# liuxinren456852/HiDeGS

Measured on NVIDIA B200. Metric: fwd+bwd Mpix/s @1M Gaussians 1080p, higher is better.
Workload: dtype f32

## Files before the change

### hidegs_b200/csrc/blend_bwd.cu

```cuda
#include "blend_common.cuh"

#include <cstdlib>
#include <mutex>

namespace hg {

namespace {

constexpr int kThreadsB = 128;


struct PixelState {
  float w[9];
  float bgT, T, acc_g, last_g, last_alpha;
  int last_contributor;
};

struct PairState {
  float2 w[9];
  float2 bgT, T, acc_g, last_g, last_alpha;
  int lastA, lastB;
};

template <int HALF>
__device__ __forceinline__ float& half_of(float2& v) { return HALF ? v.y : v.x; }
template <int HALF>
__device__ __forceinline__ float half_of(const float2& v) { return HALF ? v.y : v.x; }

template <bool GEO, bool DEPTH>
__device__ __forceinline__ void load_pixel_state(PixelState& s, bool inside, size_t pix, size_t HW, int W, int H,
                                                 float pixx, float pixy, float fx, float fy, int n,
                                                 const float* __restrict__ bg_color,
                                                 const float* __restrict__ all_map_pixels,
                                                 const float* __restrict__ final_Ts,
                                                 const uint32_t* __restrict__ n_contrib,
                                                 const float* __restrict__ dL_dpixels,
                                                 const float* __restrict__ dL_dout_all_maps,
                                                 const float* __restrict__ dL_dout_plane_depths,
                                                 const float* __restrict__ dL_invdepths) {
#pragma unroll
  for (int i = 0; i < 9; ++i) s.w[i] = 0.f;
  const float T_final = inside ? final_Ts[pix] : 0.f;
  s.last_contributor = inside ? min((int)n_contrib[pix], n) : 0;
  float bg_dot = 0.f;
  if (inside) {
#pragma unroll
    for (int c = 0; c < 3; ++c) {
      s.w[c] = dL_dpixels[c * HW + pix];
      bg_dot += __ldg(bg_color + c) * s.w[c];
    }
    if (DEPTH) s.w[3] = dL_invdepths[pix];
    if (GEO) {
#pragma unroll
      for (int c = 0; c < 5; ++c) s.w[4 + c] = dL_dout_all_maps[c * HW + pix];
      const float rayx = (float)(((double)pixx - W * 0.5) / (double)fx);
      const float rayy = (float)(((double)pixy - H * 0.5) / (double)fy);
      const float nx = all_map_pixels[pix], ny = all_map_pixels[HW + pix], nz = all_map_pixels[2 * HW + pix];
      const float dist = all_map_pixels[4 * HW + pix];
      const float tmp = (float)((double)(nx * rayx + ny * rayy + nz) + 1.0e-8);
      const float dpd = dL_dout_plane_depths[pix];
      s.w[8] += (-dpd / tmp);
      s.w[4] += dpd * (dist / (tmp * tmp) * rayx);
      s.w[5] += dpd * (dist / (tmp * tmp) * rayy);
      s.w[6] += dpd * (dist / (tmp * tmp));
    }
  }
  s.bgT = -T_final * bg_dot;
  s.T = T_final;
  s.acc_g = s.last_g = s.last_alpha = 0.f;
}

constexpr int kGroupC = 16;
constexpr int kWarpsC = kThreadsB / 32;

constexpr int kRecQuadsC = 4;
constexpr int kAStride = 68;

template <bool INTERP>
struct alignas(16) BwdMmaSmem {
  float4 rec[kWarpsC][32 * kRecQuadsC];
  alignas(16) float a_w[kWarpsC][kGroupC * kAStride];
  float a_p[kWarpsC][kGroupC * kAStride];
  float2 b_ch0[kWarpsC][8][32];
  float2 b_ch8[kWarpsC][8][4];
  float2 zero2;
  float2 b_mom[8][32];
  float2 tf[INTERP ? kWarpsC : 1][INTERP ? 32 : 1];
  uint32_t info[kWarpsC][32];
};
constexpr uint32_t kHasA = 1u << 30, kHasB = 1u << 31;
constexpr uint32_t kARowBytes = kAStride * 4;
constexpr uint32_t kAPOffset = kWarpsC * kGroupC * kAStride * 4;
constexpr uint32_t kMetaOffset = 64 * 4;

__device__ __forceinline__ void sts_v2(uint32_t addr, float a, float b) {
  asm volatile("st.shared.v2.f32 [%0], {%1, %2};" ::"r"(addr), "f"(a), "f"(b) : "memory");
}
__device__ __forceinline__ void sts_v4(uint32_t addr, float a, float b, float c, float d) {
  asm volatile("st.shared.v4.f32 [%0], {%1, %2, %3, %4};" ::"r"(addr), "f"(a), "f"(b), "f"(c), "f"(d) : "memory");
}

__device__ __forceinline__ void ldmatrix_x4(uint32_t (&r)[4], const float* smem_row_ptr) {
  const uint32_t a = (uint32_t)__cvta_generic_to_shared(smem_row_ptr);
  asm volatile("ldmatrix.sync.aligned.m8n8.x4.shared.b16 {%0,%1,%2,%3}, [%4];"
               : "=r"(r[0]), "=r"(r[1]), "=r"(r[2]), "=r"(r[3])
               : "r"(a));
}

__device__ __forceinline__ void split_tf32(float v, uint32_t& hi, uint32_t& lo) {
  asm("and.b32 %0, %1, 0xffffe000;" : "=r"(hi) : "r"(__float_as_uint(v)));
  lo = __float_as_uint(v - __uint_as_float(hi));
}

__device__ __forceinline__ void split_tf32_pair(float v0, float v1, uint32_t& hi0, uint32_t& lo0, uint32_t& hi1,
                                                uint32_t& lo1) {
  asm("and.b32 %0, %1, 0xffffe000;" : "=r"(hi0) : "r"(__float_as_uint(v0)));
  asm("and.b32 %0, %1, 0xffffe000;" : "=r"(hi1) : "r"(__float_as_uint(v1)));
  const float2 lo = __fadd2_rn(make_float2(v0, v1), make_float2(-__uint_as_float(hi0), -__uint_as_float(hi1)));
  lo0 = __float_as_uint(lo.x);
  lo1 = __float_as_uint(lo.y);
}

__device__ __forceinline__ void mma_tf32(float (&d)[4], uint32_t a0, uint32_t a1, uint32_t a2, uint32_t a3, uint32_t b0,
                                         uint32_t b1) {
  asm volatile(
      "mma.sync.aligned.m16n8k8.row.col.f32.tf32.tf32.f32 {%0,%1,%2,%3}, {%4,%5,%6,%7}, {%8,%9}, {%0,%1,%2,%3};"
      : "+f"(d[0]), "+f"(d[1]), "+f"(d[2]), "+f"(d[3])
      : "r"(a0), "r"(a1), "r"(a2), "r"(a3), "r"(b0), "r"(b1));
}

__device__ __forceinline__ void red_add_v2(float* p, float a, float b) {
  asm volatile("red.global.add.v2.f32 [%0], {%1, %2};" ::"l"(p), "f"(a), "f"(b) : "memory");
}
__device__ __forceinline__ void red_add_v4(float* p, float a, float b, float c, float d) {
  asm volatile("red.global.add.v4.f32 [%0], {%1, %2, %3, %4};" ::"l"(p), "f"(a), "f"(b), "f"(c), "f"(d) : "memory");
}

template <bool GEO, bool DEPTH, bool INTERP, bool ACC, int HALF>
__device__ __forceinline__ bool pixel_pair_c(PairState& ps, const float4 ea, const float4 eb, const float4 ec,
                                             const float4 ed, const float2 tf, float pixx, float2 neg_pixy, int q,
                                             float& wgt, float& p, float& p3, bool& near) {
  struct {
    float &T, &acc_g, &last_g, &last_alpha;
    const float bgT;
    const int last_contributor;
    float w[9];
  } s{half_of<HALF>(ps.T), half_of<HALF>(ps.acc_g), half_of<HALF>(ps.last_g), half_of<HALF>(ps.last_alpha),
      half_of<HALF>(ps.bgT), HALF ? ps.lastB : ps.lastA,
      {half_of<HALF>(ps.w[0]), half_of<HALF>(ps.w[1]), half_of<HALF>(ps.w[2]), half_of<HALF>(ps.w[3]),
       half_of<HALF>(ps.w[4]), half_of<HALF>(ps.w[5]), half_of<HALF>(ps.w[6]), half_of<HALF>(ps.w[7]),
       half_of<HALF>(ps.w[8])}};
  const float dx = __fsub_rn(ea.x, pixx), dy = __fadd_rn(ea.y, half_of<HALF>(neg_pixy));
  const float quad = __fmaf_rn(dx, __fmul_rn(dx, ea.z), __fmul_rn(dy, __fmul_rn(dy, eb.x)));
  const float power = __fmaf_rn(quad, -0.5f, -__fmul_rn(dy, __fmul_rn(dx, ea.w)));
  const float test_alpha = __fmul_rn(eb.y, expf(power));
  float blend_alpha = fminf(0.99f, test_alpha);
  float opac_mult = 1.0f;
  if (INTERP) {
    const float my_alpha = blend_alpha;
    if (ACC) {
      const float kidsqrt = 1.0f - powf(1.0f - my_alpha, tf.y);
      blend_alpha = tf.x * my_alpha + (1.0f - tf.x) * kidsqrt;
      opac_mult = tf.x - powf(1.0f - my_alpha, tf.y - 1.0f) * (tf.x - 1.0f) * tf.y;
    } else {
      const float lg = __log2f(1.0f - my_alpha);
      const float kidsqrt = 1.0f - exp2f(tf.y * lg);
      blend_alpha = tf.x * my_alpha + (1.0f - tf.x) * kidsqrt;
      opac_mult = tf.x - exp2f((tf.y - 1.0f) * lg) * (tf.x - 1.0f) * tf.y;
      near = near || fabsf(blend_alpha - 1.0f / 255.0f) < 2e-6f;
    }
  }
  const bool valid = (q < s.last_contributor) && !(power > 0.0f) && !(blend_alpha < 1.0f / 255.0f);
  const float alpha = valid ? blend_alpha : 0.f;
  float rinv;
  asm("rcp.approx.ftz.f32 %0, %1;" : "=f"(rinv) : "f"(1.0f - alpha));
  const float Tn = s.T * rinv;
  wgt = alpha * Tn;
  float g = ec.x * s.w[0] + ec.y * s.w[1] + ec.z * s.w[2];
  if (DEPTH) g += ec.w * s.w[3];
  if (GEO) {
    const float ee = eb.z;
    g += ed.x * s.w[4] + ed.y * s.w[5] + ed.z * s.w[6] + ed.w * s.w[7] + ee * s.w[8];
  }
  const float acc_new = s.last_alpha * s.last_g + (1.0f - s.last_alpha) * s.acc_g;
  const float dL_dalpha = (g - acc_new) * Tn + s.bgT * rinv;
  s.T = Tn;
  s.acc_g = acc_new;
  s.last_g = g;
  s.last_alpha = alpha;
  p = test_alpha > 0.99f ? 0.f : (INTERP ? (valid ? test_alpha : 0.f) : alpha) * dL_dalpha;
  p3 = INTERP ? opac_mult * p : 0.f;
  return valid;
}

template <bool GEO, bool DEPTH>
__device__ __forceinline__ bool pixel_pair_c2(PairState& s, const float4 ea, const float4 eb, const float4 ec,
                                              const float4 ed, float pixx, float2 neg_pixy, int q, float2& wgt,
                                              float2& p) {
  const float dx = __fsub_rn(ea.x, pixx);
  const float dxa = __fmul_rn(dx, ea.z);
  const float ndxb = __fmul_rn(dx, -ea.w);
  const float2 dy = __fadd2_rn(bc2(ea.y), neg_pixy);
  const float2 quad = __ffma2_rn(bc2(dx), bc2(dxa), __fmul2_rn(dy, __fmul2_rn(dy, bc2(eb.x))));
  const float2 power = __ffma2_rn(quad, bc2(-0.5f), __fmul2_rn(dy, bc2(ndxb)));
  const float2 test_alpha = __fmul2_rn(bc2(eb.y), expf_pair(power));
  const float bA = fminf(0.99f, test_alpha.x), bB = fminf(0.99f, test_alpha.y);
  const bool validA = (q < s.lastA) && !(power.x > 0.0f) && !(bA < 1.0f / 255.0f);
  const bool validB = (q < s.lastB) && !(power.y > 0.0f) && !(bB < 1.0f / 255.0f);
  const float2 alpha = make_float2(validA ? bA : 0.f, validB ? bB : 0.f);
  const float2 om = __ffma2_rn(alpha, bc2(-1.0f), bc2(1.0f));
  float2 rinv;
  asm("rcp.approx.ftz.f32 %0, %1;" : "=f"(rinv.x) : "f"(om.x));
  asm("rcp.approx.ftz.f32 %0, %1;" : "=f"(rinv.y) : "f"(om.y));
  const float2 Tn = __fmul2_rn(s.T, rinv);
  wgt = __fmul2_rn(alpha, Tn);
  float2 g = __ffma2_rn(bc2(ec.z), s.w[2], __ffma2_rn(bc2(ec.y), s.w[1], __fmul2_rn(bc2(ec.x), s.w[0])));
  if (DEPTH) g = __ffma2_rn(bc2(ec.w), s.w[3], g);
  if (GEO) {
    g = __ffma2_rn(bc2(ed.x), s.w[4], g);
    g = __ffma2_rn(bc2(ed.y), s.w[5], g);
    g = __ffma2_rn(bc2(ed.z), s.w[6], g);
    g = __ffma2_rn(bc2(ed.w), s.w[7], g);
    g = __ffma2_rn(bc2(eb.z), s.w[8], g);
  }
  const float2 om_last = __ffma2_rn(s.last_alpha, bc2(-1.0f), bc2(1.0f));
  const float2 acc_new = __ffma2_rn(s.last_alpha, s.last_g, __fmul2_rn(om_last, s.acc_g));
  const float2 diff = __fadd2_rn(g, make_float2(-acc_new.x, -acc_new.y));
  const float2 dL_dalpha = __ffma2_rn(diff, Tn, __fmul2_rn(s.bgT, rinv));
  s.T = Tn;
  s.acc_g = acc_new;
  s.last_g = g;
  s.last_alpha = alpha;
  p = __fmul2_rn(alpha, dL_dalpha);
  p.x = test_alpha.x > 0.99f ? 0.f : p.x;
  p.y = test_alpha.y > 0.99f ? 0.f : p.y;
  return validA || validB;
}

template <bool GEO, bool DEPTH, bool INTERP>
__global__ void __launch_bounds__(kThreadsB, INTERP ? 3 : 4)
blend_bwd3_kernel(const uint2* __restrict__ ranges, const uint32_t* __restrict__ point_list,
                  const float4* __restrict__ records, const float* __restrict__ ts, const int* __restrict__ kids,
                  const int W, const int H, const float fx, const float fy,
                  const float* __restrict__ bg_color, const float* __restrict__ all_map_pixels,
                  const float* __restrict__ final_Ts, const uint32_t* __restrict__ n_contrib,
                  const float* __restrict__ dL_dpixels, const float* __restrict__ dL_dout_all_maps,
                  const float* __restrict__ dL_dout_plane_depths, const float* __restrict__ dL_invdepths,
                  float* __restrict__ accum) {
  extern __shared__ __align__(16) unsigned char smem_raw[];
  BwdMmaSmem<INTERP>& sm = *reinterpret_cast<BwdMmaSmem<INTERP>*>(smem_raw);

  const int tid = threadIdx.x;
  const int lane = tid & 31, warp = tid >> 5;
  const uint32_t tile = blockIdx.y * gridDim.x + blockIdx.x;
  const int wx0 = blockIdx.x * HG_BLOCK_X + (warp & 1) * 8;
  const int wy0 = blockIdx.y * HG_BLOCK_Y + (warp >> 1) * 8;
  const int pxi = wx0 + (lane & 7), pyA = wy0 + (lane >> 3), pyB = pyA + 4;
  const bool insideA = pxi < W && pyA < H, insideB = pxi < W && pyB < H;
  const float pixx = (float)pxi, pixyA = (float)pyA, pixyB = (float)pyB;
  const float fx0 = (float)wx0, fx1 = (float)(wx0 + 7);
  const float2 fy0 = make_float2((float)wy0, (float)(wy0 + 4)), fy1 = make_float2((float)(wy0 + 3), (float)(wy0 + 7));
  const float cx = (float)wx0 + 3.5f, cy = (float)wy0 + 3.5f;
  const size_t HW = (size_t)H * W;

  const uint2 range = ranges[tile];
  const int n = (int)(range.y - range.x);

  PairState S;
  PixelState A, B;
  load_pixel_state<GEO, DEPTH>(A, insideA, (size_t)pyA * W + pxi, HW, W, H, pixx, pixyA, fx, fy, n, bg_color,
                               all_map_pixels, final_Ts, n_contrib, dL_dpixels, dL_dout_all_maps, dL_dout_plane_depths,
                               dL_invdepths);
  load_pixel_state<GEO, DEPTH>(B, insideB, (size_t)pyB * W + pxi, HW, W, H, pixx, pixyB, fx, fy, n, bg_color,
                               all_map_pixels, final_Ts, n_contrib, dL_dpixels, dL_dout_all_maps, dL_dout_plane_depths,
                               dL_invdepths);

#pragma unroll
  for (int c = 0; c < 9; ++c) S.w[c] = make_float2(A.w[c], B.w[c]);
  S.bgT = make_float2(A.bgT, B.bgT);
  S.T = make_float2(A.T, B.T);
  S.acc_g = S.last_g = S.last_alpha = make_float2(0.f, 0.f);
  S.lastA = A.last_contributor;
  S.lastB = B.last_contributor;
  const float2 neg_pixy = make_float2(-pixyA, -pixyB);
  int wmaxA = A.last_contributor, wmaxB = B.last_contributor;
#pragma unroll
  for (int o = 16; o > 0; o >>= 1) {
    wmaxA = max(wmaxA, __shfl_xor_sync(0xffffffffu, wmaxA, o));
    wmaxB = max(wmaxB, __shfl_xor_sync(0xffffffffu, wmaxB, o));
  }
  const int wmax = max(wmaxA, wmaxB);
  int first_id = 0;
  if (wmax - 1 - lane >= 0) first_id = (int)__ldg(point_list + range.x + (wmax - 1 - lane));

  {
    const int ks = lane >> 2, jA = 2 * (lane & 3);
    float* const ch0 = reinterpret_cast<float*>(&sm.b_ch0[warp][ks][0]);
    float* const ch8 = reinterpret_cast<float*>(&sm.b_ch8[warp][ks][0]);
    const int fa = 2 * (jA & 3) + (jA >> 2), fb = 2 * ((jA + 1) & 3) + ((jA + 1) >> 2);
#pragma unroll
    for (int c = 0; c < 8; ++c) {
      ch0[8 * c + fa] = A.w[c];
      ch0[8 * c + fb] = B.w[c];
    }
    if (GEO) {
      ch8[fa] = A.w[8];
      ch8[fb] = B.w[8];
      if (tid == 0) sm.zero2 = make_float2(0.f, 0.f);
    }
    for (int i = tid; i < 8 * 32; i += kThreadsB) {
      const int s_ = i >> 5, l_ = i & 31, g_ = l_ >> 2, t_ = l_ & 3;
      float m[2];
#pragma unroll
      for (int h = 0; h < 2; ++h) {
        const int k = 8 * s_ + t_ + 4 * h, owner = k >> 1;
        const float xi = (float)(owner & 7) - 3.5f, eta = (float)((owner >> 3) + 4 * (k & 1)) - 3.5f;
        switch (g_) {
          case 0: m[h] = 1.f; break;
          case 1: m[h] = xi; break;
          case 2: m[h] = eta; break;
          case 3: m[h] = xi * xi; break;
          case 4: m[h] = xi * eta; break;
          case 5: m[h] = eta * eta; break;
          default: m[h] = 0.f; break;
        }
      }
      sm.b_mom[s_][l_] = make_float2(m[0], m[1]);
    }
  }

  __syncthreads();
  const float ddelx_dx = 0.5f * W, ddely_dy = 0.5f * H;

  float* const a_w = sm.a_w[warp];
  float* const a_p = sm.a_p[warp];
  const int fg = lane >> 2, ft = lane & 3;
  const int a_ld = ((lane & 7) + 8 * ((lane >> 3) & 1)) * kAStride + 4 * (lane >> 4);
  const float2* const b8_src = fg == 0 ? &sm.b_ch8[warp][0][ft] : &sm.zero2;
  const int b8_step = fg == 0 ? 4 : 0;
  int rows = 0;
  uint32_t park_base;
  asm volatile("mov.u32 %0, %1;" : "=r"(park_base) : "r"((uint32_t)__cvta_generic_to_shared(a_w + 2 * lane)));

  auto flush = [&]() {
    __syncwarp();
    float dc0[4] = {0.f, 0.f, 0.f, 0.f}, dc8[4] = {0.f, 0.f, 0.f, 0.f}, dm[4] = {0.f, 0.f, 0.f, 0.f};
    float dc0x[4] = {0.f, 0.f, 0.f, 0.f}, dc8x[4] = {0.f, 0.f, 0.f, 0.f}, dmx[4] = {0.f, 0.f, 0.f, 0.f};
#pragma unroll
    for (int s_ = 0; s_ < 8; ++s_) {
      uint32_t wq[4], pq[4];
      ldmatrix_x4(wq, a_w + a_ld + 8 * s_);
      ldmatrix_x4(pq, a_p + a_ld + 8 * s_);
      uint32_t w0h, w0l, w1h, w1l, w2h, w2l, w3h, w3l, p0h, p0l, p1h, p1l, p2h, p2l, p3h, p3l;
      split_tf32_pair(__uint_as_float(wq[0]), __uint_as_float(wq[1]), w0h, w0l, w1h, w1l);
      split_tf32_pair(__uint_as_float(wq[2]), __uint_as_float(wq[3]), w2h, w2l, w3h, w3l);
      split_tf32_pair(__uint_as_float(pq[0]), __uint_as_float(pq[1]), p0h, p0l, p1h, p1l);
      split_tf32_pair(__uint_as_float(pq[2]), __uint_as_float(pq[3]), p2h, p2l, p3h, p3l);
      const float2 bq = sm.b_ch0[warp][s_][lane];
      uint32_t b0h, b0l, b1h, b1l;
      split_tf32_pair(bq.x, bq.y, b0h, b0l, b1h, b1l);
      mma_tf32(dc0, w0h, w1h, w2h, w3h, b0h, b1h);
      mma_tf32(dc0x, w0l, w1l, w2l, w3l, b0h, b1h);
      mma_tf32(dc0x, w0h, w1h, w2h, w3h, b0l, b1l);
      if (GEO) {
        const float2 b8 = b8_src[s_ * b8_step];
        split_tf32_pair(b8.x, b8.y, b0h, b0l, b1h, b1l);
        mma_tf32(dc8, w0h, w1h, w2h, w3h, b0h, b1h);
        mma_tf32(dc8x, w0l, w1l, w2l, w3l, b0h, b1h);
        mma_tf32(dc8x, w0h, w1h, w2h, w3h, b0l, b1l);
      }
      const float2 bm = sm.b_mom[s_][lane];
      mma_tf32(dm, p0h, p1h, p2h, p3h, __float_as_uint(bm.x), __float_as_uint(bm.y));
      mma_tf32(dmx, p0l, p1l, p2l, p3l, __float_as_uint(bm.x), __float_as_uint(bm.y));
    }
#pragma unroll
    for (int i = 0; i < 4; ++i) {
      dc0[i] += dc0x[i];
      dc8[i] += dc8x[i];
      dm[i] += dmx[i];
    }
    float Sy[2], Sxx[2], Sxy[2], Syy[2];
#pragma unroll
    for (int h = 0; h < 2; ++h) {
      Sy[h] = __shfl_down_sync(0xffffffffu, dm[2 * h], 1);
      Sxx[h] = __shfl_down_sync(0xffffffffu, dm[2 * h + 1], 1);
      Sxy[h] = __shfl_down_sync(0xffffffffu, dm[2 * h], 2);
      Syy[h] = __shfl_down_sync(0xffffffffu, dm[2 * h + 1], 2);
    }
#pragma unroll
    for (int h = 0; h < 2; ++h) {
      const int row = fg + 8 * h;
      if (row < rows) {
        const float4 m1 = *reinterpret_cast<const float4*>(a_p + row * kAStride + 64);
        float* const arow = accum + (size_t)__float_as_int(m1.w) * HG_ACC_FLOATS;
        red_add_v2(arow + 2 * ft, dc0[2 * h], dc0[2 * h + 1]);
        if (ft == 0) {
          const float4 m0 = *reinterpret_cast<const float4*>(a_w + row * kAStride + 64);
          const float S1 = dm[2 * h], Sx = dm[2 * h + 1];
          const float u = m0.x - cx, v = m0.y - cy, o = m1.y;
          const float Dx = u * S1 - Sx, Dy = v * S1 - Sy[h];
          const float Qxx = u * (Dx - Sx) + Sxx[h];
          const float Qxy = u * Dy - v * Sx + Sxy[h];
          const float Qyy = v * (Dy - Sy[h]) + Syy[h];
          const float g9 = -ddelx_dx * (m0.z * Dx + m0.w * Dy);
          const float g10 = -ddely_dy * (m1.x * Dy + m0.w * Dx);
          red_add_v4(arow + 8, dc8[2 * h], g9, g10, -0.5f * Qxx);
          red_add_v2(arow + 12, -0.5f * Qxy, -0.5f * Qyy);
          atomicAdd(arow + 14, __fdividef(INTERP ? m1.z : S1, o));
        }
      }
    }
    rows = 0;
    __syncwarp();
  };

  float4* const w_rec = sm.rec[warp];
  uint32_t* const w_info = sm.info[warp];
  const uint32_t lanes_below = (1u << lane) - 1u;
  Prefetch pf;
  auto prefetch = [&](int base) {
    const int q = base - lane;
    if (q >= 0) gather_record<INTERP>(pf, point_list, records, ts, kids, range.x + q);
  };
  if (wmax - 1 - lane >= 0) gather_record_id<INTERP>(pf, first_id, records, ts, kids);

  for (int base = wmax - 1; base >= 0; base -= 32) {
    const int q_mine = base - lane;
    bool keepA = false, keepB = false;
    const float a = pf.r0.z, bb = pf.r0.w, c = pf.r1.x, o = pf.r1.y;
    if (q_mine >= 0) {
      const float tau = cull_tau(a, bb, c, o, INTERP);
      may_touch2(pf.r0.x, pf.r0.y, a, bb, c, tau, fx0, fx1, fy0, fy1, keepA, keepB);
      keepA = keepA && q_mine < wmaxA;
      keepB = keepB && q_mine < wmaxB;
    }
    const uint32_t maskA = __ballot_sync(0xffffffffu, keepA), maskB = __ballot_sync(0xffffffffu, keepB);
    const uint32_t mask = maskA | maskB;
    if (keepA || keepB) {
      const int slot = __popc(mask & lanes_below);
      float4* d = w_rec + kRecQuadsC * slot;
      d[0] = pf.r0;
      d[1] = make_float4(c, o, pf.r3.z, __int_as_float(pf.id));
      d[2] = make_float4(pf.r1.z, pf.r1.w, pf.r2.x, pf.r2.y);
      if (GEO) d[3] = make_float4(pf.r2.z, pf.r2.w, pf.r3.x, pf.r3.y);
      if (INTERP) sm.tf[warp][slot] = make_float2(pf.it, pf.ifrac);
      w_info[slot] = (uint32_t)q_mine | (keepA ? kHasA : 0u) | (keepB ? kHasB : 0u);
    }
    __syncwarp();
    if (base >= 32) prefetch(base - 32);
    const int cnt = __popc(mask);
    for (int i = 0; i < cnt; ++i) {
      const float4* e = w_rec + kRecQuadsC * i;
      const uint32_t info = w_info[i];
      const float4 ea = e[0];
      const float4 eb = e[1];
      const float4 ec = e[2];      float4 ed = make_float4(0.f, 0.f, 0.f, 0.f);
      if (GEO) ed = e[3];
      float2 tf = make_float2(1.f, 1.f);
      if (INTERP) tf = sm.tf[warp][i];
      const int q = (int)(info & (kHasA - 1u));
      const bool hasA = (info & kHasA) != 0u, hasB = (info & kHasB) != 0u;
      float wA = 0.f, pA = 0.f, wB = 0.f, pB = 0.f, p3A = 0.f, p3B = 0.f;
      bool any, near = false;
      const float2 S_T = S.T, S_acc = S.acc_g, S_lg = S.last_g, S_la = S.last_alpha;
      if (hasA && hasB) {
        if (!INTERP) {
          float2 w2, p2;
          any = pixel_pair_c2<GEO, DEPTH>(S, ea, eb, ec, ed, pixx, neg_pixy, q, w2, p2);
          wA = w2.x; wB = w2.y; pA = p2.x; pB = p2.y;
        } else {
          any = pixel_pair_c<GEO, DEPTH, INTERP, false, 0>(S, ea, eb, ec, ed, tf, pixx, neg_pixy, q, wA, pA, p3A, near);
          any |= pixel_pair_c<GEO, DEPTH, INTERP, false, 1>(S, ea, eb, ec, ed, tf, pixx, neg_pixy, q, wB, pB, p3B, near);
        }
      } else if (hasA) {
        any = pixel_pair_c<GEO, DEPTH, INTERP, false, 0>(S, ea, eb, ec, ed, tf, pixx, neg_pixy, q, wA, pA, p3A, near);
      } else {
        any = pixel_pair_c<GEO, DEPTH, INTERP, false, 1>(S, ea, eb, ec, ed, tf, pixx, neg_pixy, q, wB, pB, p3B, near);
      }
      if (INTERP && __any_sync(0xffffffffu, near)) {
        S.T = S_T; S.acc_g = S_acc; S.last_g = S_lg; S.last_alpha = S_la;
        wA = pA = wB = pB = p3A = p3B = 0.f;
        any = false;
        if (hasA) any = pixel_pair_c<GEO, DEPTH, INTERP, true, 0>(S, ea, eb, ec, ed, tf, pixx, neg_pixy, q, wA, pA, p3A, near);
        if (hasB) any |= pixel_pair_c<GEO, DEPTH, INTERP, true, 1>(S, ea, eb, ec, ed, tf, pixx, neg_pixy, q, wB, pB, p3B, near);
      }
      if (__ballot_sync(0xffffffffu, any) == 0) continue;
      float s3 = eb.z;
      if (INTERP) {
        s3 = p3A + p3B;
#pragma unroll
        for (int o = 16; o > 0; o >>= 1) s3 += __shfl_xor_sync(0xffffffffu, s3, o);
      }
      const uint32_t row_addr = park_base + rows * kARowBytes;
      sts_v2(row_addr, wA, wB);
      sts_v2(row_addr + kAPOffset, pA, pB);
      if (lane == 0) {
        sts_v4(row_addr + kMetaOffset, ea.x, ea.y, ea.z, ea.w);
        sts_v4(row_addr + kAPOffset + kMetaOffset, eb.x, eb.y, s3, eb.w);
      }
      if (++rows == kGroupC) flush();
    }
    __syncwarp();
  }
  if (rows > 0) flush();
}

}

int launch_blend_bwd(const hg_raster_inputs& in, const GeomState& g, const BinState& b,
                     const ImageState& img, dim3 grid, float focal_x, float focal_y,
                     const float* all_map_pixels, const float* dL_dpix,
                     const float* dL_dout_all_map, const float* dL_dout_plane_depth,
                     const float* dL_dout_invdepth, float* accum, cudaStream_t stream) {
  const bool interp = in.ts != nullptr && in.kids != nullptr;
  const bool geo = in.render_geo != 0;
  const bool depth = dL_dout_invdepth != nullptr;
    static std::mutex attr_mu;
    static bool attr_done[64] = {}, attr_ok[64] = {};
    int device = 0;
    HG_CUDA_TRY(cudaGetDevice(&device));
    if (device < 0 || device >= 64) {
      set_error("blend_bwd: device index %d out of range", device);
      return HG_ERR_CUDA;
    }
    {
      std::lock_guard<std::mutex> lk(attr_mu);
      if (!attr_done[device]) {
        bool ok = true;
        const int b0 = (int)sizeof(BwdMmaSmem<false>), b1 = (int)sizeof(BwdMmaSmem<true>);
        const auto attr = cudaFuncAttributeMaxDynamicSharedMemorySize;
        ok &= cudaFuncSetAttribute(blend_bwd3_kernel<true, true, false>, attr, b0) == cudaSuccess;
        ok &= cudaFuncSetAttribute(blend_bwd3_kernel<true, false, false>, attr, b0) == cudaSuccess;
        ok &= cudaFuncSetAttribute(blend_bwd3_kernel<false, true, false>, attr, b0) == cudaSuccess;
        ok &= cudaFuncSetAttribute(blend_bwd3_kernel<false, false, false>, attr, b0) == cudaSuccess;
        ok &= cudaFuncSetAttribute(blend_bwd3_kernel<true, true, true>, attr, b1) == cudaSuccess;
        ok &= cudaFuncSetAttribute(blend_bwd3_kernel<true, false, true>, attr, b1) == cudaSuccess;
        ok &= cudaFuncSetAttribute(blend_bwd3_kernel<false, true, true>, attr, b1) == cudaSuccess;
        ok &= cudaFuncSetAttribute(blend_bwd3_kernel<false, false, true>, attr, b1) == cudaSuccess;
        attr_ok[device] = ok;
        attr_done[device] = true;
      }
    }
    if (!attr_ok[device]) {
      set_error("blend_bwd: could not reserve %zu bytes of shared memory", sizeof(BwdMmaSmem<true>));
      return HG_ERR_CUDA;
    }
#define HG_LAUNCH3(G_, D_, I_)                                                                            \
  blend_bwd3_kernel<G_, D_, I_><<<grid, kThreadsB, sizeof(BwdMmaSmem<I_>), stream>>>(                     \
      img.ranges, b.vals, g.records, in.ts, in.kids, in.W, in.H, focal_x, focal_y, in.background,         \
      all_map_pixels, img.final_T, img.n_contrib, dL_dpix, dL_dout_all_map, dL_dout_plane_depth,          \
      dL_dout_invdepth, accum)
    if (interp) {
      if (geo && depth) HG_LAUNCH3(true, true, true);
      else if (geo) HG_LAUNCH3(true, false, true);
      else if (depth) HG_LAUNCH3(false, true, true);
      else HG_LAUNCH3(false, false, true);
    } else {
      if (geo && depth) HG_LAUNCH3(true, true, false);
      else if (geo) HG_LAUNCH3(true, false, false);
      else if (depth) HG_LAUNCH3(false, true, false);
      else HG_LAUNCH3(false, false, false);
    }
#undef HG_LAUNCH3
  HG_POST_LAUNCH(in.debug, stream, "blend_bwd");
  return HG_OK;
}

}
```

Baseline: 1054.

## Split non-interp backward pair blend into classify and recurrence, processing two records per step

For the non-interpolating backward path, the per-Gaussian pair evaluation is split into a state-independent classify step (exp, validity, colour dot product) and a short serial recurrence step. Two records are classified back-to-back before their recurrences are folded, giving more instruction-level parallelism on the dependent transmittance chain. The >0.99 saturation flag is encoded in the sign of the stored alpha so it no longer needs to be carried separately. The unrolled step must stop at the park-group boundary, which adds control-flow and register pressure, and hasA/hasB masking now comes from the info bits.

```diff
diff --git a/hidegs_b200/csrc/blend_bwd.cu b/hidegs_b200/csrc/blend_bwd.cu
--- a/hidegs_b200/csrc/blend_bwd.cu
+++ b/hidegs_b200/csrc/blend_bwd.cu
@@ -194,9 +194,10 @@
 }
 
 template <bool GEO, bool DEPTH>
-__device__ __forceinline__ bool pixel_pair_c2(PairState& s, const float4 ea, const float4 eb, const float4 ec,
-                                              const float4 ed, float pixx, float2 neg_pixy, int q, float2& wgt,
-                                              float2& p) {
+__device__ __forceinline__ bool classify_pair(const PairState& s, const float4 ea, const float4 eb, const float4 ec,
+                                              const float4 ed, float pixx, float2 neg_pixy, uint32_t info,
+                                              float2& alpha_s, float2& g) {
+  const uint32_t qA = (info & ~kHasB) ^ kHasA, qB = (info & ~kHasA) ^ kHasB;
   const float dx = __fsub_rn(ea.x, pixx);
   const float dxa = __fmul_rn(dx, ea.z);
   const float ndxb = __fmul_rn(dx, -ea.w);
@@ -205,16 +206,11 @@
   const float2 power = __ffma2_rn(quad, bc2(-0.5f), __fmul2_rn(dy, bc2(ndxb)));
   const float2 test_alpha = __fmul2_rn(bc2(eb.y), expf_pair(power));
   const float bA = fminf(0.99f, test_alpha.x), bB = fminf(0.99f, test_alpha.y);
-  const bool validA = (q < s.lastA) && !(power.x > 0.0f) && !(bA < 1.0f / 255.0f);
-  const bool validB = (q < s.lastB) && !(power.y > 0.0f) && !(bB < 1.0f / 255.0f);
-  const float2 alpha = make_float2(validA ? bA : 0.f, validB ? bB : 0.f);
-  const float2 om = __ffma2_rn(alpha, bc2(-1.0f), bc2(1.0f));
-  float2 rinv;
-  asm("rcp.approx.ftz.f32 %0, %1;" : "=f"(rinv.x) : "f"(om.x));
-  asm("rcp.approx.ftz.f32 %0, %1;" : "=f"(rinv.y) : "f"(om.y));
-  const float2 Tn = __fmul2_rn(s.T, rinv);
-  wgt = __fmul2_rn(alpha, Tn);
-  float2 g = __ffma2_rn(bc2(ec.z), s.w[2], __ffma2_rn(bc2(ec.y), s.w[1], __fmul2_rn(bc2(ec.x), s.w[0])));
+  const bool validA = (qA < (uint32_t)s.lastA) && !(power.x > 0.0f) && !(bA < 1.0f / 255.0f);
+  const bool validB = (qB < (uint32_t)s.lastB) && !(power.y > 0.0f) && !(bB < 1.0f / 255.0f);
+  const float aA = validA ? bA : 0.f, aB = validB ? bB : 0.f;
+  alpha_s = make_float2(test_alpha.x > 0.99f ? -aA : aA, test_alpha.y > 0.99f ? -aB : aB);
+  g = __ffma2_rn(bc2(ec.z), s.w[2], __ffma2_rn(bc2(ec.y), s.w[1], __fmul2_rn(bc2(ec.x), s.w[0])));
   if (DEPTH) g = __ffma2_rn(bc2(ec.w), s.w[3], g);
   if (GEO) {
     g = __ffma2_rn(bc2(ed.x), s.w[4], g);
@@ -223,18 +219,27 @@
     g = __ffma2_rn(bc2(ed.w), s.w[7], g);
     g = __ffma2_rn(bc2(eb.z), s.w[8], g);
   }
-  const float2 om_last = __ffma2_rn(s.last_alpha, bc2(-1.0f), bc2(1.0f));
-  const float2 acc_new = __ffma2_rn(s.last_alpha, s.last_g, __fmul2_rn(om_last, s.acc_g));
+  return validA || validB;
+}
+
+__device__ __forceinline__ void recur_pair(PairState& s, float2 alpha_s, float2 g, float2& wgt, float2& p) {
+  const float2 alpha = make_float2(fabsf(alpha_s.x), fabsf(alpha_s.y));
+  const float2 om = __ffma2_rn(alpha, bc2(-1.0f), bc2(1.0f));
+  float2 rinv;
+  asm("rcp.approx.ftz.f32 %0, %1;" : "=f"(rinv.x) : "f"(om.x));
+  asm("rcp.approx.ftz.f32 %0, %1;" : "=f"(rinv.y) : "f"(om.y));
+  const float2 Tn = __fmul2_rn(s.T, rinv);
+  wgt = __fmul2_rn(alpha, Tn);
+  const float2 last_alpha = make_float2(fabsf(s.last_alpha.x), fabsf(s.last_alpha.y));
+  const float2 om_last = __ffma2_rn(last_alpha, bc2(-1.0f), bc2(1.0f));
+  const float2 acc_new = __ffma2_rn(last_alpha, s.last_g, __fmul2_rn(om_last, s.acc_g));
   const float2 diff = __fadd2_rn(g, make_float2(-acc_new.x, -acc_new.y));
   const float2 dL_dalpha = __ffma2_rn(diff, Tn, __fmul2_rn(s.bgT, rinv));
   s.T = Tn;
   s.acc_g = acc_new;
   s.last_g = g;
-  s.last_alpha = alpha;
-  p = __fmul2_rn(alpha, dL_dalpha);
-  p.x = test_alpha.x > 0.99f ? 0.f : p.x;
-  p.y = test_alpha.y > 0.99f ? 0.f : p.y;
-  return validA || validB;
+  s.last_alpha = alpha_s;
+  p = __fmul2_rn(make_float2(fmaxf(alpha_s.x, 0.f), fmaxf(alpha_s.y, 0.f)), dL_dalpha);
 }
 
 template <bool GEO, bool DEPTH, bool INTERP>
@@ -449,7 +454,44 @@
     __syncwarp();
     if (base >= 32) prefetch(base - 32);
     const int cnt = __popc(mask);
-    for (int i = 0; i < cnt; ++i) {
+    if (!INTERP) {
+      auto fold_park = [&](float2 a, float2 g, const float4& ea, const float4& eb) {
+        float2 w, p;
+        recur_pair(S, a, g, w, p);
+        const uint32_t row_addr = park_base + rows * kARowBytes;
+        sts_v2(row_addr, w.x, w.y);
+        sts_v2(row_addr + kAPOffset, p.x, p.y);
+        if (lane == 0) {
+          sts_v4(row_addr + kMetaOffset, ea.x, ea.y, ea.z, ea.w);
+          sts_v4(row_addr + kAPOffset + kMetaOffset, eb.x, eb.y, eb.z, eb.w);
+        }
+        ++rows;
+      };
+      for (int i = 0; i < cnt;) {
+        const float4* e0 = w_rec + kRecQuadsC * i;
+        const float4 ea0 = e0[0], eb0 = e0[1], ec0 = e0[2], ed0 = GEO ? e0[3] : make_float4(0.f, 0.f, 0.f, 0.f);
+        float2 a0, g0;
+        if (i + 1 < cnt) {
+          const float4* e1 = e0 + kRecQuadsC;
+          const float4 ea1 = e1[0], eb1 = e1[1], ec1 = e1[2], ed1 = GEO ? e1[3] : make_float4(0.f, 0.f, 0.f, 0.f);
+          float2 a1, g1;
+          const bool any0 = classify_pair<GEO, DEPTH>(S, ea0, eb0, ec0, ed0, pixx, neg_pixy, w_info[i], a0, g0);
+          const bool any1 = classify_pair<GEO, DEPTH>(S, ea1, eb1, ec1, ed1, pixx, neg_pixy, w_info[i + 1], a1, g1);
+          const bool keep0 = __ballot_sync(0xffffffffu, any0) != 0u;
+          const bool keep1 = __ballot_sync(0xffffffffu, any1) != 0u;
+          if (keep0) fold_park(a0, g0, ea0, eb0);
+          const bool take1 = rows < kGroupC;
+          if (take1 && keep1) fold_park(a1, g1, ea1, eb1);
+          i += take1 ? 2 : 1;
+        } else {
+          const bool any0 = classify_pair<GEO, DEPTH>(S, ea0, eb0, ec0, ed0, pixx, neg_pixy, w_info[i], a0, g0);
+          if (__ballot_sync(0xffffffffu, any0) != 0u) fold_park(a0, g0, ea0, eb0);
+          ++i;
+        }
+        if (rows == kGroupC) flush();
+      }
+    }
+    for (int i = 0; INTERP && i < cnt; ++i) {
       const float4* e = w_rec + kRecQuadsC * i;
       const uint32_t info = w_info[i];
       const float4 ea = e[0];
@@ -464,14 +506,8 @@
       bool any, near = false;
       const float2 S_T = S.T, S_acc = S.acc_g, S_lg = S.last_g, S_la = S.last_alpha;
       if (hasA && hasB) {
-        if (!INTERP) {
-          float2 w2, p2;
-          any = pixel_pair_c2<GEO, DEPTH>(S, ea, eb, ec, ed, pixx, neg_pixy, q, w2, p2);
-          wA = w2.x; wB = w2.y; pA = p2.x; pB = p2.y;
-        } else {
-          any = pixel_pair_c<GEO, DEPTH, INTERP, false, 0>(S, ea, eb, ec, ed, tf, pixx, neg_pixy, q, wA, pA, p3A, near);
-          any |= pixel_pair_c<GEO, DEPTH, INTERP, false, 1>(S, ea, eb, ec, ed, tf, pixx, neg_pixy, q, wB, pB, p3B, near);
-        }
+        any = pixel_pair_c<GEO, DEPTH, INTERP, false, 0>(S, ea, eb, ec, ed, tf, pixx, neg_pixy, q, wA, pA, p3A, near);
+        any |= pixel_pair_c<GEO, DEPTH, INTERP, false, 1>(S, ea, eb, ec, ed, tf, pixx, neg_pixy, q, wB, pB, p3B, near);
       } else if (hasA) {
         any = pixel_pair_c<GEO, DEPTH, INTERP, false, 0>(S, ea, eb, ec, ed, tf, pixx, neg_pixy, q, wA, pA, p3A, near);
       } else {
```

After: 1073 (median of 6 runs). +1.7%, better.
